# fusiyuan2010/CSC

Hardware: AMD Instinct MI355X
Metric: encode MB/s (10^6 input bytes / wall-clock) on enwik9 stand-in, -m3 -d64m; stream bit-exact vs reference (higher is better)
Workload: dtype u8/u32 (byte + 32-bit integer work; 12-bit probabilities, 64-bit range-coder low)

## Files before the change

csc_amd/csrc/csc_kernels.hip:

```cpp
#include <hip/hip_runtime.h>
#include <stdint.h>
#include <stdlib.h>

#include "csc_device.h"
#include "csc_tables.h"

namespace cscmi {

#define DEV __device__ __forceinline__
#define GLOBAL_AS __attribute__((address_space(1)))
typedef GLOBAL_AS uint8_t gu8;
typedef GLOBAL_AS uint16_t gu16;
typedef GLOBAL_AS uint32_t gu32;
typedef uint32_t __attribute__((ext_vector_type(4))) raw_vec4;
typedef GLOBAL_AS raw_vec4 gvec4;
#define UNI(x) ((uint32_t)__builtin_amdgcn_readfirstlane((int)(x)))

#ifndef CSCMI_TU
#define CSCMI_TU 0
#endif
static __device__ __constant__ uint32_t d_p2bits[512];
static __device__ __constant__ uint32_t d_logtable[513];

__device__ static const uint32_t kDltIndex[5] = {1, 2, 3, 4, 8};
// ... 9 lines not shown
struct DpShared {
    uint32_t cmd, idle;
    uint32_t dec;
    uint32_t price_done, relax_done;
    uint32_t ins_done, erep_done;
    uint32_t lp_int;
    uint32_t abort, gate;
    uint32_t wpos0, pos0, aplimit, limit0, stage_base, stage_end;
    uint32_t bstat[2];
    DpEdge e[2];
    uint16_t st_lit[64], st_p1[64];
    uint32_t e2[4][8];
    uint32_t er[4][8];
};
struct EncLds {
    uint32_t P[P_COUNT + 4];
    uint16_t p2b[512];
    uint32_t len_price[32], len_price_old[32];
    uint32_t rep[4];
    union {
        uint32_t cd2[kDpWaves][32];
        struct { uint32_t cd2_row0[32]; uint32_t cmp_pos[16], cmp_lim[16], cmp_res[16]; };
    };
    uint32_t rp42[kDpWaves][4];
    uint32_t rg_price[256], rg_dist[256];
    uint32_t rg_rep[256 * 4];
    uint16_t rg_back[256];
    uint8_t rg_state[256];
    union {
        struct {
            uint32_t fin_dist[kAPLimit + 1];
            uint16_t fin_back[kAPLimit + 2];
            union {
                uint16_t fin_next[kAPLimit + 2];
                struct { uint32_t appt_price[256], appt_dist[256]; };
            };
            uint8_t fin_lit[kAPLimit + 3];
        };
        uint32_t fin2[(kAPLimit + 1) * 2];
        struct { uint16_t trie_next[300 * 26]; uint8_t trie_sym[304]; };
        struct {
            uint2 tok[kTokRing];
            uint32_t pipe_cmd, pipe_ack, tok_head, tok_tail;
            uint32_t hand[16];
        };
    };
    DpShared dp;
    uint32_t stage[(kMinBlock + 64) / 4];
};

struct Sc {
    EncState *S;
    EncLds *L;
    void *X;
    struct CoderQ *Q;
    uint32_t q_head, q_room;
    gu8 *wnd;
    uint32_t wnd_size, vld_rge;
    gu32 *ht2, *ht3, *ht6, *bt_head, *bt_nodes, *p_lit, *p_delta, *mfbuf;
    uint32_t ht6_off, bth_off;
    bool fast_ht;
    uint32_t pr_off, pr_rmask, pr_pol;
    uint32_t gm6, gm2, gm3, gmb, gslot;
    uint32_t ht_bits, ht_width, ht_low, ht_cyc, bt_bits, bt_size, bt_cyc, good_len;
    uint32_t lz_good_len, lz_bt_cyc, lz_ht_cyc;
    uint32_t bt_pos, pos, wnd_curpos;
    uint32_t state, ctx, lp_rebuild_int;
    uint64_t rc_low;
    uint32_t rc_range, rc_cache, rc_cachesize, rc_size, bc_size, bc_curbits, bc_curval, bsize;
    gu8 *rc_buf, *bc_buf, *arena, *swapbuf;
    uint32_t arena_used, arena_cap, error;
    uint32_t lane;
    uint32_t stage_base, stage_end;
    uint32_t cand_len_v, cand_dist_v;
    uint32_t wv, dp_seq, dp_idle, dp_seq_seen;
    uint32_t st_find, st_slide, st_bt, st_lit, st_match;
    uint32_t pipe_ok, piped, tok_headl, tok_tail_seen, pipe_seq, pair_ok;
#ifdef CSCMI_TIMERS
    unsigned long long tm[16];
#endif
};

#ifdef CSCMI_TIMERS
#define TM_DECL unsigned long long tm__ = __builtin_readcyclecounter()
#define TM_ADD(c, k) do { unsigned long long n__ = __builtin_readcyclecounter(); (c).tm[k] += n__ - tm__; tm__ = n__; } while (0)
#define TM_RESET tm__ = __builtin_readcyclecounter()
#ifdef CSCMI_TIMERS_FINE
#define TMF_ADD(c, k) TM_ADD(c, k)
#else
#define TMF_ADD(c, k) do {} while (0)
#endif
#else
#define TMF_ADD(c, k) do {} while (0)
#define TM_DECL do {} while (0)
#define TM_ADD(c, k) do {} while (0)
#define TM_RESET do {} while (0)
#endif

DEV uint32_t umin(uint32_t a, uint32_t b) { return a < b ? a : b; }
DEV uint64_t uni64(uint64_t v) { return ((uint64_t)UNI((uint32_t)(v >> 32)) << 32) | UNI((uint32_t)v); }
template <class T> DEV T *uni_gptr(T *p) { return (T *)(uintptr_t)uni64((uint64_t)(uintptr_t)p); }
DEV void sc_uniform(Sc &c)
{
    c.S = uni_gptr(c.S); c.wnd = uni_gptr(c.wnd); c.wnd_size = UNI(c.wnd_size); c.vld_rge = UNI(c.vld_rge);
    c.ht2 = uni_gptr(c.ht2); c.ht3 = uni_gptr(c.ht3); c.ht6 = uni_gptr(c.ht6); c.bt_head = uni_gptr(c.bt_head); c.bt_nodes = uni_gptr(c.bt_nodes);
    c.p_lit = uni_gptr(c.p_lit); c.p_delta = uni_gptr(c.p_delta); c.mfbuf = uni_gptr(c.mfbuf);
    c.ht6_off = UNI(c.ht6_off); c.bth_off = UNI(c.bth_off);
    c.ht_bits = UNI(c.ht_bits); c.ht_width = UNI(c.ht_width); c.ht_low = UNI(c.ht_low); c.ht_cyc = UNI(c.ht_cyc);
    c.bt_bits = UNI(c.bt_bits); c.bt_size = UNI(c.bt_size); c.bt_cyc = UNI(c.bt_cyc); c.good_len = UNI(c.good_len);
    c.lz_good_len = UNI(c.lz_good_len); c.lz_bt_cyc = UNI(c.lz_bt_cyc); c.lz_ht_cyc = UNI(c.lz_ht_cyc);
    c.bt_pos = UNI(c.bt_pos); c.pos = UNI(c.pos); c.wnd_curpos = UNI(c.wnd_curpos);
    c.state = UNI(c.state); c.ctx = UNI(c.ctx); c.lp_rebuild_int = UNI(c.lp_rebuild_int);
    c.rc_low = uni64(c.rc_low); c.rc_range = UNI(c.rc_range); c.rc_cache = UNI(c.rc_cache); c.rc_cachesize = UNI(c.rc_cachesize);
    c.rc_size = UNI(c.rc_size); c.bc_size = UNI(c.bc_size); c.bc_curbits = UNI(c.bc_curbits); c.bc_curval = UNI(c.bc_curval); c.bsize = UNI(c.bsize);
    c.rc_buf = uni_gptr(c.rc_buf); c.bc_buf = uni_gptr(c.bc_buf); c.arena = uni_gptr(c.arena); c.swapbuf = uni_gptr(c.swapbuf);
    c.arena_used = UNI(c.arena_used); c.arena_cap = UNI(c.arena_cap); c.error = UNI(c.error);
    c.stage_base = UNI(c.stage_base); c.stage_end = UNI(c.stage_end);
    c.wv = UNI(c.wv); c.dp_seq = UNI(c.dp_seq); c.dp_idle = UNI(c.dp_idle); c.dp_seq_seen = UNI(c.dp_seq_seen);
    c.st_find = UNI(c.st_find); c.st_slide = UNI(c.st_slide); c.st_bt = UNI(c.st_bt); c.st_lit = UNI(c.st_lit); c.st_match = UNI(c.st_match);
    c.q_head = UNI(c.q_head); c.q_room = UNI(c.q_room);
}

DEV void wave_fence() { __builtin_amdgcn_fence(__ATOMIC_SEQ_CST, "workgroup"); }
DEV uint32_t rdlane(uint32_t v, uint32_t lane) { return (uint32_t)__builtin_amdgcn_readlane((int)v, (int)lane); }
DEV uint32_t wrlane(uint32_t val, uint32_t lane, uint32_t old) { return (threadIdx.x & 63u) == lane ? val : old; }

DEV uint64_t load8u(const gu8 *p)
{
    uintptr_t a = (uintptr_t)p;
    uint32_t sh = (uint32_t)a & 3u;
    const gu32 *q = (const gu32 *)(a & ~(uintptr_t)3);
    uint32_t d0 = q[0], d1 = q[1], d2 = q[2];
    uint32_t lo = __builtin_amdgcn_alignbyte(d1, d0, sh);
    uint32_t hi = __builtin_amdgcn_alignbyte(d2, d1, sh);
    return ((uint64_t)hi << 32) | lo;
}
DEV uint32_t ldb(const gu8 *p) { return UNI((uint32_t)*p); }

DEV uint64_t stage_load8(const uint32_t *stage, uint32_t byte_idx)
{
    uint32_t sh = byte_idx & 3u;
    const uint32_t *q = stage + (byte_idx >> 2);
    uint32_t d0 = q[0], d1 = q[1], d2 = q[2];
    uint32_t lo = __builtin_amdgcn_alignbyte(d1, d0, sh);
    uint32_t hi = __builtin_amdgcn_alignbyte(d2, d1, sh);
    return ((uint64_t)hi << 32) | lo;
}


__device__ __noinline__ void lanes_copy16(gvec4 *d4, const gvec4 *s4, uint32_t n16)
{
    for (uint32_t i = threadIdx.x & 63u; i < n16; i += 64) d4[i] = s4[i];
}
__device__ __noinline__ void lanes_copy8(gu8 *dst, const gu8 *src, uint32_t n)
{
    for (uint32_t t = threadIdx.x & 63u; t < n; t += 64) dst[t] = src[t];
}
__device__ __noinline__ void lanes_fill32(gu32 *dst, uint32_t n, uint32_t v)
{
    for (uint32_t t = threadIdx.x & 63u; t < n; t += 64) dst[t] = v;
}
__device__ __noinline__ void lanes_stage(uint8_t *sb, const gu8 *src, uint32_t first, uint32_t end)
{
    for (uint32_t t = first + (threadIdx.x & 63u); t < end; t += 64) sb[t] = src[t];
}
DEV void emit_block(Sc &c, uint32_t kind, const gu8 *buf, uint32_t size)
{
    uint32_t need = 16 + ((size + 15) & ~15u);
    if (c.arena_used + need > c.arena_cap) { c.error = ERR_ARENA_FULL; return; }
    gu8 *dst = c.arena + c.arena_used;
    wave_fence();
    ((gu32 *)dst)[0] = kind; ((gu32 *)dst)[1] = size;
    lanes_copy16((gvec4 *)(dst + 16), (const gvec4 *)buf, (size + 15) >> 4);
    c.arena_used += need;
}

constexpr uint32_t kCoderQ = 4096;
constexpr uint32_t kPDumpE = P_COUNT + 3;
struct CoderQ {
    uint32_t pub, tail, done, pad;
    uint32_t e[kCoderQ];
};
DEV void q_publish(Sc &c)
{
    __builtin_amdgcn_fence(__ATOMIC_RELEASE, "workgroup", "local");
    *(volatile __attribute__((address_space(3))) uint32_t *)&c.Q->pub = c.q_head;
}
DEV void q_publish_to(Sc &c, uint32_t to)
{
    __builtin_amdgcn_fence(__ATOMIC_RELEASE, "workgroup", "local");
    *(volatile __attribute__((address_space(3))) uint32_t *)&c.Q->pub = to;
}
constexpr uint32_t ERR_QUEUE_STALL = 0x40200000u;
DEV uint32_t q_wait_room(Sc &c, uint32_t need)
{
    uint32_t used, spins = 0;
    if (__builtin_expect(c.error != 0, 0)) return 0;
    while ((used = c.q_head - UNI(*(volatile __attribute__((address_space(3))) uint32_t *)&c.Q->tail)) > kCoderQ - need) {
        __builtin_amdgcn_s_sleep(2);
        if (++spins > (1u << 24)) { if (!c.error) c.error = ERR_QUEUE_STALL | (used & 0xFFFFu); return 0; }
    }
    return used;
}
DEV void q_push(Sc &c, uint32_t e)
{
    if (__builtin_expect(c.q_room == 0, 0)) {
        q_publish(c);
        c.q_room = umin(kCoderQ - 64u - q_wait_room(c, 128u), 256u);
    }
    c.Q->e[c.q_head & (kCoderQ - 1)] = e;
    c.q_head++; c.q_room--;
}

DEV void q_push_bits(Sc &c, uint32_t pold, uint32_t bit, uint32_t n, uint32_t from = 0)
{
    if (__builtin_expect(c.q_room < n, 0)) {
        q_publish(c);
        c.q_room = umin(kCoderQ - 64u - q_wait_room(c, 128u), 256u);
    }
    const uint32_t k = c.lane - from;
    c.Q->e[(c.q_head + (k < n ? k : 63u)) & (kCoderQ - 1)] = 0x80000000u | (bit ? 0x1000u : 0u) | pold;
    c.q_head += n; c.q_room -= n;
}

DEV void rc_put(Sc &c, uint32_t byte)
{
    c.rc_buf[c.rc_size++] = (uint8_t)byte;
    if (c.rc_size == c.bsize) { emit_block(c, 1, c.rc_buf, c.bsize); c.rc_size = 0; }
}

DEV void rc_shift_low(Sc &c)
{
    uint32_t low32 = (uint32_t)c.rc_low, top = (uint32_t)(c.rc_low >> 32);
    if (low32 < 0xFF000000u || top != 0) {
        uint32_t temp = c.rc_cache;
        do {
            rc_put(c, (temp + top) & 0xFF);
            temp = 0xFF;
        } while (--c.rc_cachesize != 0);
        c.rc_cache = low32 >> 24;
    }
    c.rc_cachesize++;
    c.rc_low = (uint64_t)(low32 << 8);
}

DEV void rc_code(Sc &c, uint32_t v, uint32_t p)
{
    if (c.Q) { q_push(c, 0x80000000u | (v ? 0x1000u : 0u) | p); return; }
    const uint32_t bound = (c.rc_range >> 12) * p;
    c.rc_low += v ? 0u : bound;
    c.rc_range = v ? bound : c.rc_range - bound;
    if (__builtin_expect(c.rc_range < (1u << 24), 0)) { c.rc_range <<= 8; rc_shift_low(c); }
}
DEV uint32_t p_update(uint32_t v, uint32_t p) { return v ? p + ((0xFFFu - p) >> 5) : p - (p >> 5); }

DEV void enc_bit_lds(Sc &c, uint32_t v, uint32_t idx)
{
    uint32_t p = UNI(c.L->P[idx]);
    c.L->P[idx] = p_update(v, p);
    rc_code(c, v, p);
}

DEV void bc_put(Sc &c, uint32_t byte)
{
    c.bc_buf[c.bc_size++] = (uint8_t)byte;
    if (c.bc_size == c.bsize) { emit_block(c, 0, c.bc_buf, c.bsize); c.bc_size = 0; }
}

DEV void enc_direct16(Sc &c, uint32_t val, uint32_t len)
{
    if (c.Q) { q_push(c, 0x40000000u | (len << 16) | (val & 0xFFFFu)); return; }
    c.bc_curval = (c.bc_curval << len) | val;
    c.bc_curbits += len;
    while (c.bc_curbits >= 8) {
        bc_put(c, (c.bc_curval >> (c.bc_curbits - 8)) & 0xFF);
        c.bc_curbits -= 8;
    }
}
DEV void enc_direct(Sc &c, uint32_t v, uint32_t l)
{
    if (l <= 16) enc_direct16(c, v, l);
    else { enc_direct16(c, v >> 16, l - 16); enc_direct16(c, v & 0xFFFF, 16); }
}

DEV void coder_flush(Sc &c)
{
    if (c.Q) { q_push(c, 0x20000000u); q_publish(c); return; }
    for (int i = 0; i < 5; i++) rc_shift_low(c);
    c.rc_size++;
    bc_put(c, (c.bc_curval << (8 - c.bc_curbits)) & 0xFF);
    bc_put(c, 0);
    emit_block(c, 1, c.rc_buf, c.rc_size);
    emit_block(c, 0, c.bc_buf, c.bc_size);
    c.rc_low = 0; c.rc_range = 0xFFFFFFFFu; c.rc_cachesize = 1; c.rc_cache = 0;
    c.rc_size = c.bc_size = 0; c.bc_curbits = c.bc_curval = 0;
}


DEV uint32_t bit_price(const Sc &c, uint32_t v, uint32_t p)
{
    return UNI(c.L->p2b[(v ? p : 4096u - p) >> 3]);
}
DEV uint32_t lds_price(const Sc &c, uint32_t v, uint32_t idx) { return bit_price(c, v, UNI(c.L->P[idx])); }

DEV void encode_int(Sc &c, uint32_t num)
{
    uint32_t slot = num ? 31u - (uint32_t)__builtin_clz(num) : 0u;
    enc_direct(c, slot, 5);
    if (slot == 0) enc_direct(c, num, 1);
    else enc_direct(c, num - (1u << slot), slot);
}

DEV void encode_matchlen_1(Sc &c, uint32_t len)
{
    if (len < 16) {
        uint32_t base;
        if (len < 8) { enc_bit_lds(c, 0, P_LEN_SLOT); base = P_LEN_X1; }
// ... 370 lines not shown
```

csc_amd/csrc/csc_kernels_blocks.inc:

```


DEV uint32_t e89_xswap(uint32_t x)
{
    x <<= 7;
    return (x >> 24) | (((x >> 16) & 0xFFu) << 8) | (((x >> 8) & 0xFFu) << 16) | ((x & 0xFFu) << (24 - 7));
}
DEV void flt_forward_e89(Sc &c, gu8 *src, uint32_t size)
{
    uint32_t next_ok = 0;
    for (uint32_t base = 0; base + 5 < size; base += 64) {
        uint32_t j0 = base + c.lane;
        bool cand = false;
        if (j0 + 5 < size) cand = (src[j0] & 0xFEu) == 0xE8u;
        uint64_t m = __ballot(cand);
        while (m) {
            uint32_t bit = (uint32_t)__builtin_ctzll(m);
            m &= m - 1;
            uint32_t j = base + bit;
            if (j < next_ok) continue;
            next_ok = j + 4;
            uint64_t v = load8u(src + j + 1);
            uint32_t x = UNI((uint32_t)v) - 0xFF000000u;
            if (x < 0x02000000u) {
                x = (x + (j + 5)) & 0x01FFFFFFu;
                x = e89_xswap(x) + 0xFF000000u;
                src[j + 1] = (uint8_t)x; src[j + 2] = (uint8_t)(x >> 8);
                src[j + 3] = (uint8_t)(x >> 16); src[j + 4] = (uint8_t)(x >> 24);
            }
        }
        wave_fence();
    }
}

DEV void flt_forward_delta(Sc &c, gu8 *src, uint32_t size, uint32_t chn)
{
    if (size < 512) return;
    gu8 *copy = c.swapbuf;
    for (uint32_t t = c.lane; t < size; t += 64) copy[t] = src[t];
    wave_fence();
    for (uint32_t j = c.lane; j < size; j += 64) {
        uint32_t ch = j % chn, idx = j / chn;
        uint32_t dst = idx;
        for (uint32_t k = 0; k < ch; k++) dst += (size - k + chn - 1) / chn;
        uint32_t prev = 0;
        if (idx > 0) prev = copy[j - chn];
        else if (ch > 0) {
            uint32_t nprev = (size - (ch - 1) + chn - 1) / chn;
            prev = copy[(ch - 1) + (nprev - 1) * chn];
        }
        src[dst] = (uint8_t)(copy[j] - prev);
    }
    wave_fence();
}

DEV uint32_t umax16(uint32_t a, uint32_t b) { return a > b ? a : b; }
DEV uint32_t flt_compose(uint32_t A, uint32_t B) { return __builtin_amdgcn_perm(0u, B, A); }
DEV uint32_t flt_forward_dict(Sc &c, gu8 *src, uint32_t size)
{
    if (size < 16384) return 0;
    EncLds *L = c.L;
    EncState *S = c.S;
    gu8 *dst = c.swapbuf;
    const uint32_t n5 = size - 5;
    for (uint32_t i = c.lane; i < 300 * 26; i += 64) L->trie_next[i] = S->trie_next[i];
    for (uint32_t i = c.lane; i < 300; i += 64) L->trie_sym[i] = S->trie_sym[i];
    uint32_t s_in = 0, dst_size = 0, p = 0;
    const uint64_t lower = (1ull << c.lane) - 1ull;
    uint64_t v8n = load8u(src + c.lane);
    for (uint32_t base = 0; base < n5; base += 64) {
        const uint32_t i = base + c.lane;
        const bool valid = i < n5;
        const uint64_t v8 = v8n;
        if (base + 64 < n5) v8n = load8u(src + i + 64);
        const uint32_t b = (uint32_t)v8 & 0xFFu;
        uint32_t sym = 0, adv = 1;
        if (valid && b >= 'a' && b <= 'z') {
            uint32_t node = 0;
            for (uint32_t j = 0; j < 8;) {
                const uint32_t idx = ((uint32_t)(v8 >> (8u * j)) & 0xFFu) - 'a';
                if (idx > 25) break;
                const uint32_t nx = L->trie_next[node * 26 + idx];
                if (nx == 0) break;
                node = nx;
                j++;
                const uint32_t ws = L->trie_sym[node];
                if (ws) { sym = ws; adv = j; }
            }
        }
        uint32_t inc = valid ? (((adv - 1u) & 3u) | 0x02010000u) : 0x03020100u;
#pragma unroll
        for (int o = 1; o < 64; o <<= 1) {
            const uint32_t t = (uint32_t)__shfl_up((int)inc, o);
            inc = (int)c.lane >= o ? flt_compose(t, inc) : inc;
        }
        const uint32_t prev = (uint32_t)__shfl_up((int)inc, 1);
        const uint32_t sb = c.lane == 0 ? s_in : (prev >> (8u * s_in)) & 3u;
        const bool mine = valid && sb == 0;
        const uint64_t on = __ballot(mine);
        const bool two = mine && sym == 0 && b >= 0x82;
        const uint64_t m2 = __ballot(two);
        const uint32_t off = dst_size + (uint32_t)__builtin_popcountll(on & lower) + (uint32_t)__builtin_popcountll(m2 & lower);
        if (mine) {
            if (sym) dst[off] = (uint8_t)sym;
            else if (two) { dst[off] = 254; dst[off + 1] = (uint8_t)b; }
            else dst[off] = (uint8_t)b;
        }
        dst_size += (uint32_t)__builtin_popcountll(on) + (uint32_t)__builtin_popcountll(m2);
        const uint32_t vcount = umin(64u, n5 - base);
        s_in = (rdlane(inc, vcount - 1) >> (8u * s_in)) & 3u;
        p = base + vcount + s_in;
    }
    wave_fence();
    for (uint32_t i = p; i < size; i++) {
        uint32_t b = ldb(src + i);
        if (b >= 0x82) { dst[dst_size++] = 254; dst[dst_size++] = (uint8_t)b; }
        else dst[dst_size++] = (uint8_t)b;
    }
    if ((double)dst_size > (double)size * 0.82) return 0;
    wave_fence();
    {
        const uint32_t full = dst_size & ~15u, up = (size + 15u) & ~15u;
        const gvec4 *s4 = (const gvec4 *)dst;
        gvec4 *d4 = (gvec4 *)src;
        raw_vec4 blanks; blanks.x = blanks.y = blanks.z = blanks.w = 0x20202020u;
        for (uint32_t t = c.lane * 16u; t < full; t += 1024u) d4[t >> 4] = s4[t >> 4];
        for (uint32_t t = full + c.lane; t < umin(full + 16u, size); t += 64) src[t] = t < dst_size ? dst[t] : (uint8_t)0x20;
        for (uint32_t t = full + 16u + c.lane * 16u; t + 16u <= size; t += 1024u) d4[t >> 4] = blanks;
        for (uint32_t t = umax16(full + 16u, size & ~15u) + c.lane; t < size; t += 64) src[t] = (uint8_t)0x20;
        (void)up;
    }
    wave_fence();
    return 1;
}

#if CSCMI_TU != 2
template <int WHICH>
__device__ __noinline__ uint32_t flt_dp4_nl(EncState *S, gu8 *swapbuf, gu8 *src, uint32_t size, uint32_t chn)
{
    Sc c;
    c.S = S; c.L = &g_lds4.base; c.swapbuf = swapbuf; c.lane = threadIdx.x & 63u;
    if (WHICH == 0) { flt_forward_e89(c, src, size); return 0; }
    if (WHICH == 1) return flt_forward_dict(c, src, size);
    flt_forward_delta(c, src, size, chn);
    return 0;
}
#endif
template <int PARSER, int FORM>
DEV void enc_compress_block(Sc &c, gu8 *src, uint32_t size, uint32_t type)
{
    if (size == 0) return;
    uint32_t mode = c.S->lz_mode;
    const bool is_dlt = type >= DT_DLT && type < DT_DLT + 5;
    if (type == DT_NORMAL) {
        encode_int(c, type);
    } else if (type == DT_EXE) {
        encode_int(c, type);
#if CSCMI_TU != 2
        if (FORM == 2) (void)flt_dp4_nl<0>(uni_gptr(c.S), uni_gptr(c.swapbuf), uni_gptr(src), UNI(size), 0);
        else
#endif
        flt_forward_e89(c, src, size);
    } else if (type == DT_ENGTXT) {
        TM_DECL;
        uint32_t ok;
#if CSCMI_TU != 2
        if (FORM == 2) ok = UNI(flt_dp4_nl<1>(uni_gptr(c.S), uni_gptr(c.swapbuf), uni_gptr(src), UNI(size), 0));
        else
#endif
        ok = flt_forward_dict(c, src, size);
        TM_ADD(c, 8);
        c.S->dict_result = ok;
        if (ok) { encode_int(c, type); encode_int(c, size); }
        else encode_int(c, DT_NORMAL);
    } else if (type == DT_FAST) {
        encode_int(c, DT_NORMAL);
    } else if (type == DT_BAD || type == DT_ENTROPY || is_dlt) {
        encode_int(c, type);
        mode = 5;
    } else {
        c.error = ERR_BAD_TYPE;
        return;
    }
    lz_encode_normal<PARSER, FORM>(c, src, size, mode);
    if (type == DT_BAD) compress_bad(c, src, size);
    else if (type == DT_ENTROPY) compress_literals(c, src, size);
    else if (is_dlt) {
#if CSCMI_TU != 2
        if (FORM == 2) (void)flt_dp4_nl<2>(uni_gptr(c.S), uni_gptr(c.swapbuf), uni_gptr(src), UNI(size), kDltIndex[type - DT_DLT]);
        else
#endif
        flt_forward_delta(c, src, size, kDltIndex[type - DT_DLT]);
        compress_rle(c, src, size);
    }
}

DEV bool dev_is_duplicate(Sc &c, const gu8 *src, uint32_t size)
{
    wave_fence();
    const uint32_t wpos = c.wnd_curpos, vld = c.vld_rge, wsz = c.wnd_size;
    for (uint32_t base = 0; base < size; base += 64) {
        const uint32_t i = base + c.lane;
        bool hit = false;
        if (i < size) {
            const uint64_t v = load8u(src + i);
            const uint32_t lo = (uint32_t)v, hi2 = (uint32_t)(v >> 32) & 0xFFFFu;
            if ((hash2_of(lo) & 15u) == 0) {
                const uint32_t hv = hash6_mul(lo, hi2);
                const uint32_t limit = size - i;
                uint32_t d[2] = {0xFFFFFFFFu, 0xFFFFFFFFu};
                if (c.ht_width) d[0] = c.pos - c.ht6[(size_t)(hv >> (32 - c.ht_bits)) * c.ht_width];
                if (c.bt_head) d[1] = c.pos - c.bt_head[hv >> (32 - c.bt_bits)];
#pragma unroll
                for (int k = 0; k < 2; k++) {
                    const uint32_t dist = d[k];
                    if (dist >= vld) continue;
                    const uint32_t cp = wpos >= dist ? wpos - dist : wpos + wsz - dist;
                    const uint32_t climit = umin(limit, wsz - cp);
                    if (climit <= 18) continue;
                    const gu8 *q = c.wnd + cp;
                    const bool e0 = load8u(src + i) == load8u(q), e1 = load8u(src + i + 8) == load8u(q + 8);
                    const uint64_t t2 = (load8u(src + i + 16) ^ load8u(q + 16)) & 0xFFFFFFull;
                    hit = hit || (e0 && e1 && t2 == 0);
                }
            }
        }
        if (__ballot(hit)) return true;
    }
    return false;
}

struct SegWalk { uint32_t csize, i, blk, last_type, last_begin, last_size, bpb; };
DEV void seg_start(SegWalk &w, uint32_t csize) { w.csize = csize; w.i = 0; w.blk = 0; w.last_type = DT_NORMAL; w.last_begin = 0; w.last_size = 0; w.bpb = 0; }
DEV bool seg_next(Sc &c, SegWalk &w, uint32_t &type, uint32_t &off, uint32_t &size, uint32_t &tail)
{
    EncState *S = c.S;
    const gu8 *src = (const gu8 *)S->inbuf;
    const uint32_t ff = S->filt_flags;
    const BlockInfo *binfo = S->binfo;
    while (w.i < w.csize) {
        const uint32_t cur = umin(kMinBlock, w.csize - w.i);
        uint32_t this_type = DT_NORMAL;
        if (ff) {
            this_type = UNI(binfo[w.blk].type);
            if (this_type != DT_SKIP) w.bpb = UNI(binfo[w.blk].bpb);
        }
        if (this_type == DT_SKIP) this_type = w.last_type;
        if (this_type != DT_NORMAL) {
            if (this_type == DT_EXE && !(ff & 4u)) this_type = DT_NORMAL;
            else if (this_type == DT_ENGTXT && !(ff & 2u)) this_type = DT_NORMAL;
            else if (this_type >= DT_DLT && !(ff & 1u)) this_type = DT_NORMAL;
        }
        if (this_type >= DT_DLT && (double)UNI(binfo[w.blk].dlt_bpb[this_type - DT_DLT]) >= w.bpb * 0.95) this_type = DT_NORMAL;
        if (this_type >= DT_NO_LZ && dev_is_duplicate(c, src + w.i, cur)) this_type = DT_NORMAL;
        const bool close = (w.last_type != this_type || w.last_size + cur > S->raw_blocksize) && w.last_size;
        if (w.last_type != this_type || w.last_size + cur > S->raw_blocksize) {
            type = w.last_type; off = w.last_begin; size = w.last_size; tail = 0;
            w.last_begin = w.i;
            w.last_size = 0;
        }
        w.last_type = this_type;
        w.last_size += cur;
        w.i += cur;
        w.blk++;
        if (close) return true;
    }
    if (w.last_size) { type = w.last_type; off = w.last_begin; size = w.last_size; tail = 1; w.last_size = 0; return true; }
    return false;
}

DEV void sc_load_regs(Sc &c, EncState *S, EncLds *L)
{
    const GLOBAL_AS EncState *G = (const GLOBAL_AS EncState *)S;
    c.S = S; c.L = L; c.X = nullptr; c.Q = nullptr; c.q_head = 0; c.q_room = 0;
    c.lane = threadIdx.x & 63;
    c.wnd = (gu8 *)G->wnd; c.wnd_size = G->wnd_size; c.vld_rge = G->vld_rge;
    c.ht2 = (gu32 *)G->ht2; c.ht3 = (gu32 *)G->ht3; c.ht6 = (gu32 *)G->ht6; c.bt_head = (gu32 *)G->bt_head; c.bt_nodes = (gu32 *)G->bt_nodes;
    c.p_lit = (gu32 *)G->p_lit; c.p_delta = (gu32 *)G->p_delta; c.swapbuf = (gu8 *)G->swapbuf;
    c.mfbuf = (gu32 *)G->mfbuf;
    c.ht6_off = kHT2Size + kHT3Size;
    c.bth_off = c.ht6_off + (G->ht_width << G->ht_bits);
    {
        uint32_t wd = G->ht_width < G->lz_ht_cyc ? G->ht_width : G->lz_ht_cyc;
        c.gm6 = c.lane < wd ? 0xFFFFFFFFu : 0u;
        c.gm2 = c.lane == 32 ? 0xFFFFFFFFu : 0u;
        c.gm3 = c.lane == 33 ? 0xFFFFFFFFu : 0u;
        c.gmb = (c.lane == 34 && G->bt_head) ? 0xFFFFFFFFu : 0u;
// ... 505 lines not shown
```

csc_amd/csrc/csc_kernels_lz.inc:

```

DEV void lz_encode_nonlit(Sc &c, uint32_t ulen, uint32_t udist)
{
    EncLds *L = c.L;
    if (udist <= 4) {
        if (ulen == 1 && udist == 1) encode_rep0len1(c);
        else {
            encode_rep_match(c, udist - 1, ulen - 2);
            uint32_t d = UNI(L->rep[udist - 1]);
            for (uint32_t k = udist - 1; k > 0; k--) L->rep[k] = UNI(L->rep[k - 1]);
            L->rep[0] = d;
        }
    } else {
        encode_match(c, udist - 5, ulen - 2);
        uint32_t r0 = UNI(L->rep[0]), r1 = UNI(L->rep[1]), r2 = UNI(L->rep[2]);
        L->rep[3] = r2; L->rep[2] = r1; L->rep[1] = r0; L->rep[0] = udist - 4;
    }
}

typedef volatile __attribute__((address_space(3))) uint32_t lds_vu32;
DEV uint32_t lds_vload(uint32_t *p) { return UNI(*(lds_vu32 *)p); }
DEV void lds_vstore(uint32_t *p, uint32_t v) { *(lds_vu32 *)p = v; }
DEV void lds_release() { __builtin_amdgcn_fence(__ATOMIC_RELEASE, "workgroup"); }
DEV void lds_acquire() { __builtin_amdgcn_fence(__ATOMIC_ACQUIRE, "workgroup"); }

// ... 184 lines not shown
            encode_match(c, nd - 5, next - i - 2);
            c.ctx = UNI(L->fin_lit[next - 1]);
        }
        i = next;
    }
    L->rep[c.lane & 3u] = L->rg_rep[(end & 255u) * 4 + (c.lane & 3u)];
}

DEV void lz_compress_advanced(Sc &c, uint32_t size)
{
    EncLds *L = c.L;
    size = UNI(size);
    for (uint32_t i = 0; i < size;) {
        sc_uniform(c);
        i = UNI(i);
        uint32_t a0l = 1, a0d = 0;
        uint32_t apcur = 0, apend = 1;
        const uint32_t aplimit = umin(kAPLimit, size - i);
        for (;;) {
            TM_DECL;
            const uint32_t sidx = c.wnd_curpos - c.stage_base + 16;
            uint64_t v9 = stage_load8(L->stage, sidx - 1);
            const uint32_t b01 = UNI((uint32_t)v9), b45 = UNI((uint32_t)(v9 >> 32));
            const uint32_t lit_ctx = c.wnd_curpos ? (b01 & 0xFFu) : 0u;
            const uint32_t cur_lit = (b01 >> 8) & 0xFFu;
            const MfPre pre = mf_pre(c, (b01 >> 8) | (b45 << 24), b45 >> 8);
            const uint32_t lk = c.lane & 7, lcc = cur_lit | 0x100u;
            const uint32_t plit_raw = c.p_lit[lit_ctx * 256 + (lcc >> (8 - lk))];
            const uint32_t slot = apcur & 255u;
            uint32_t cur_state, r0, r1, r2, r3, base_price;
            if (apcur) {
                cur_state = UNI(L->rg_state[slot]);
                r0 = UNI(L->rg_rep[slot * 4 + 0]); r1 = UNI(L->rg_rep[slot * 4 + 1]);
                r2 = UNI(L->rg_rep[slot * 4 + 2]); r3 = UNI(L->rg_rep[slot * 4 + 3]);
                base_price = UNI(L->rg_price[slot]);
                L->fin_dist[apcur] = UNI(L->rg_dist[slot]);
                L->fin_back[apcur] = (uint16_t)UNI(L->rg_back[slot]);
            } else {
                cur_state = c.state;
                r0 = UNI(L->rep[0]); r1 = UNI(L->rep[1]); r2 = UNI(L->rep[2]); r3 = UNI(L->rep[3]);
                base_price = 0;
                L->rg_price[0] = 0;
                L->fin_back[0] = 0;
                L->rg_rep[0] = r0; L->rg_rep[1] = r1; L->rg_rep[2] = r2; L->rg_rep[3] = r3;
            }
            L->fin_lit[apcur] = (uint8_t)cur_lit;
            bool has1 = false;
            uint32_t p1 = 0, lane_dist = 0, lane_price = 0, t_lit0 = 0;
            if (apcur < aplimit) {
                TM_ADD(c, 4);
                mf_find_priced(c, cur_state, c.wnd_curpos, size - i - apcur, pre, r0, r1, r2, r3, a0l, a0d, has1, p1, lane_dist, lane_price, t_lit0);
                TM_RESET;
            }
            uint32_t exit_kind = 0;
            if (apcur == 0 && a0d == 0) exit_kind = 2;
            else if (apcur == aplimit) exit_kind = 1;
            else if (a0l == 1 && apcur + 1 == apend) exit_kind = 2;
            else {
                if (apcur + 1 >= apend) { L->rg_price[apend & 255u] = 0xFFFFFFFFu; apend++; }
                if (a0l >= c.lz_good_len || (a0l > 1 && a0l + apcur >= aplimit)) exit_kind = 3;
            }
            if (exit_kind) {
                lz_ap_backward(c, apcur);
                i += apcur;
                if (exit_kind == 2) {
                    encode_literal(c, cur_lit);
                    c.wnd_curpos++;
                    i++;
                } else if (exit_kind == 3) {
                    lz_encode_nonlit(c, a0l, a0d);
                    mf_slide_pos(c, c.wnd_curpos, a0l, size - i);
                    i += a0l;
                    c.wnd_curpos += a0l;
                    c.ctx = stage_byte(c, c.wnd_curpos - 1);
                }
                TM_ADD(c, 6);
                break;
            }
            uint32_t cprice;
            {
                uint32_t bit = (lcc >> (7 - lk)) & 1;
                uint32_t pr = L->p2b[(bit ? plit_raw : 4096u - plit_raw) >> 3];
                pr += dpp_row_shr<1>(0, pr);
                pr += dpp_row_shr<2>(0, pr);
                pr += dpp_row_shr<4>(0, pr);
                cprice = rdlane(pr, 7) + t_lit0;
            }
            const uint32_t s1slot = (apcur + 1) & 255u;
            uint32_t nprice = UNI(L->rg_price[s1slot]);
            uint32_t n_dist = 0xFFFFFFFFu;
            if (cprice + base_price < nprice) { nprice = cprice + base_price; n_dist = 0; }
            if (has1 && p1 + base_price < nprice) { nprice = p1 + base_price; n_dist = 1; }
            if (n_dist != 0xFFFFFFFFu) {
                L->rg_dist[s1slot] = n_dist;
                L->rg_back[s1slot] = (uint16_t)apcur;
                L->rg_price[s1slot] = nprice;
                L->rg_state[s1slot] = (uint8_t)((cur_state * 4 + (n_dist ? 2 : 0)) & 0x3F);
                L->rg_rep[s1slot * 4 + 0] = r0; L->rg_rep[s1slot * 4 + 1] = r1;
                L->rg_rep[s1slot * 4 + 2] = r2; L->rg_rep[s1slot * 4 + 3] = r3;
            }
            const uint32_t len = a0l;
            if (apcur + len >= apend) {
                for (uint32_t t0 = apend; t0 <= apcur + len; t0 += 64) L->rg_price[umin(t0 + c.lane, apcur + len) & 255u] = 0xFFFFFFFFu;
                apend = apcur + len + 1;
            }
            for (uint32_t l0 = 2; l0 <= len; l0 += 64) {
                const uint32_t ll = l0 + c.lane;
                const bool in = ll <= len;
                const uint32_t lli = in ? ll : 2u;
                const uint32_t ad = l0 == 2 ? lane_dist : L->appt_dist[lli];
                const uint32_t pr = l0 == 2 ? lane_price : L->appt_price[lli];
                const uint32_t t0 = (apcur + ll) & 255u;
                const uint32_t was = L->rg_price[t0];
                const bool win = in & (ad != 0) & (pr + base_price < was);
                const uint32_t t = win ? t0 : slot;
                L->rg_dist[t] = ad;
                L->rg_back[t] = (uint16_t)apcur;
                L->rg_price[t] = pr + base_price;
                const bool isrep = ad <= 4;
                const uint32_t rsel0 = L->cd2[c.wv][(ad - 1) & 3u];
                const uint32_t ns = (cur_state * 4 + (isrep ? 3u : 1u)) & 0x3F;
                const uint32_t n0 = isrep ? rsel0 : ad - 4;
                const uint32_t n1 = (isrep && ad == 1) ? r1 : r0;
                const uint32_t n2 = (isrep && ad <= 2) ? r2 : r1;
                const uint32_t n3 = (isrep && ad <= 3) ? r3 : r2;
                L->rg_state[t] = (uint8_t)ns;
                L->rg_rep[t * 4 + 0] = n0; L->rg_rep[t * 4 + 1] = n1; L->rg_rep[t * 4 + 2] = n2; L->rg_rep[t * 4 + 3] = n3;
            }
            apcur++;
            c.wnd_curpos++;
            TM_ADD(c, 5);
        }
    }
}

DEV void lz_compress_advanced_dp4(Sc &c, uint32_t size);
DEV void d4_master_call(Sc &c, uint32_t size);
DEV void lz_compress_advanced_bt(Sc &c, uint32_t size);
DEV void bt_parser_call(Sc &c, uint32_t size);
DEV bool bt_ok(const Sc &c, uint32_t size);
DEV void lz_compress_normal_hp(Sc &c, uint32_t size, bool lazy);
DEV void hp_parser_call(Sc &c, uint32_t size, bool lazy);
DEV bool hp_ok(const Sc &c);

template <int PARSER, int FORM>
DEV void lz_encode_normal(Sc &c, const gu8 *src, uint32_t size, uint32_t lz_mode)
{
    const bool two_waves = PARSER == 2 && lz_mode != 5 && c.pipe_ok;
    if (two_waves) pipe_begin(c);
    for (uint32_t i = 0; i < size;) {
        uint32_t cur = umin(c.wnd_size - c.wnd_curpos, size - i);
        cur = umin(cur, kMinBlock);
        {
            gu8 *dst = c.wnd + c.wnd_curpos;
            const gu8 *s = src + i;
            TM_DECL;
            lanes_copy8(dst, s, cur);
            wave_fence();
            c.stage_base = c.wnd_curpos;
            c.stage_end = c.wnd_curpos + cur + 40;
            uint32_t first = c.wnd_curpos >= 16 ? 0u : 16u - c.wnd_curpos;
            uint8_t *sb = (uint8_t *)c.L->stage;
            lanes_stage(sb, c.wnd + c.wnd_curpos - 16, first, cur + 16 + 48);
            TM_ADD(c, 9);
        }
        if (lz_mode == 5) {
            mf_slide_pos_fast(c, c.wnd_curpos, cur);
            c.wnd_curpos += cur;
        } else {
            if (PARSER == 3) {
                if (FORM == 3 && bt_ok(c, cur)) bt_parser_call(c, cur);
                else if (FORM == 2 && c.pair_ok && c.pos < 0xFFFF0000u) d4_master_call(c, cur);
                else lz_compress_advanced(c, cur);
            }
            else if (FORM == 4 && hp_ok(c)) hp_parser_call(c, cur, lz_mode == 2);
            else lz_compress_normal(c, cur, lz_mode == 2);
        }
        if (c.wnd_curpos >= c.wnd_size) c.wnd_curpos = 0;
        i += cur;
    }
    if (lz_mode != 5) {
        if (c.piped) tok_push(c, TOK_NONLIT_KEEPCTX | (2u << 16), 64 + 5);
        else encode_match(c, 64, 0);
    }
    if (two_waves) pipe_end(c);
}
```

Baseline: 2.912.

## Vectorize window/stage copy and restructure dictionary filter with DPP scan and packed trie

```diff
diff --git a/csc_amd/csrc/csc_kernels.hip b/csc_amd/csrc/csc_kernels.hip
--- a/csc_amd/csrc/csc_kernels.hip
+++ b/csc_amd/csrc/csc_kernels.hip
@@ -185,17 +185,79 @@
 {
     for (uint32_t i = threadIdx.x & 63u; i < n16; i += 64) d4[i] = s4[i];
 }
-__device__ __noinline__ void lanes_copy8(gu8 *dst, const gu8 *src, uint32_t n)
-{
-    for (uint32_t t = threadIdx.x & 63u; t < n; t += 64) dst[t] = src[t];
+DEV raw_vec4 load16u(const gu8 *p)
+{
+    const uintptr_t a = (uintptr_t)p;
+    const uint32_t sh = (uint32_t)a & 3u;
+    const gu32 *q = (const gu32 *)(a & ~(uintptr_t)3);
+    const uint32_t d0 = q[0], d1 = q[1], d2 = q[2], d3 = q[3], d4 = sh ? q[4] : 0u;
+    raw_vec4 v;
+    v.x = __builtin_amdgcn_alignbyte(d1, d0, sh); v.y = __builtin_amdgcn_alignbyte(d2, d1, sh);
+    v.z = __builtin_amdgcn_alignbyte(d3, d2, sh); v.w = __builtin_amdgcn_alignbyte(d4, d3, sh);
+    return v;
+}
+constexpr int kCopyBatch = 8;
+DEV void lanes_copy16_far(gvec4 *__restrict__ d4, const gvec4 *__restrict__ s4, uint32_t n16)
+{
+    const uint32_t lane = threadIdx.x & 63u;
+    for (uint32_t u0 = 0; u0 < n16; u0 += 64u * kCopyBatch) {
+        raw_vec4 v[kCopyBatch];
+#pragma unroll
+        for (int k = 0; k < kCopyBatch; k++) v[k] = s4[umin(u0 + 64u * k + lane, n16 - 1u)];
+#pragma unroll
+        for (int k = 0; k < kCopyBatch; k++) {
+            const uint32_t u = u0 + 64u * k + lane;
+            if (u < n16) d4[u] = v[k];
+        }
+    }
+}
+constexpr int kStageBatch = 4;
+__device__ __noinline__ void lanes_copy_stage(gu8 *__restrict__ wnd, const gu8 *__restrict__ src, uint8_t *sb, uint32_t wpos, uint32_t first, uint32_t n)
+{
+    const uint32_t lane = threadIdx.x & 63u;
+    gu8 *dst = wnd + wpos;
+    const uint32_t j = lane < 16u ? lane : n + lane;
+    const bool around = lane >= 16u || lane >= first;
+    uint8_t ab = 0;
+    if (around) ab = (wnd + wpos - 16)[j];
+    const uint32_t sn16 = n >> 4;
+    const uint32_t st = (sn16 << 4) + lane;
+    uint8_t stb = 0;
+    if (lane < 16u && st < n) stb = src[st];
+    const uint32_t head = umin(n, (16u - (wpos & 15u)) & 15u), cn16 = (n - head) >> 4;
+    const uint32_t ct = head + (cn16 << 4) + (lane - 16u);
+    uint8_t hb = 0;
+    if (lane < head) hb = src[lane];
+    else if (lane >= 16u && lane < 32u && ct < n) hb = src[ct];
+    typedef __attribute__((address_space(3), aligned(8))) raw_vec4 lvec4;
+    static_assert(alignof(EncLds) % 8 == 0 && offsetof(EncLds, stage) % 8 == 0, "the stage's 16-byte units are written as two aligned 8-byte halves");
+    typedef __attribute__((address_space(3))) uint8_t lu8;
+    lu8 *sl = (lu8 *)sb;
+    lvec4 *s4 = (lvec4 *)(sl + 16);
+    gvec4 *d4 = (gvec4 *)(dst + head);
+    const gu8 *csrc = src + head;
+    for (uint32_t u0 = lane; u0 < sn16; u0 += 64u * kStageBatch) {
+        raw_vec4 v[kStageBatch];
+#pragma unroll
+        for (int k = 0; k < kStageBatch; k++) v[k] = load16u(src + umin(u0 + 64u * k, sn16 - 1u) * 16u);
+#pragma unroll
+        for (int k = 0; k < kStageBatch; k++) if (u0 + 64u * k < sn16) s4[u0 + 64u * k] = v[k];
+    }
+    if (around) sl[j] = ab;
+    if (lane < 16u && st < n) sl[16u + st] = stb;
+    for (uint32_t u0 = lane; u0 < cn16; u0 += 64u * kStageBatch) {
+        raw_vec4 v[kStageBatch];
+#pragma unroll
+        for (int k = 0; k < kStageBatch; k++) v[k] = load16u(csrc + umin(u0 + 64u * k, cn16 - 1u) * 16u);
+#pragma unroll
+        for (int k = 0; k < kStageBatch; k++) if (u0 + 64u * k < cn16) d4[u0 + 64u * k] = v[k];
+    }
+    if (lane < head) dst[lane] = hb;
+    else if (lane >= 16u && lane < 32u && ct < n) dst[ct] = hb;
 }
 __device__ __noinline__ void lanes_fill32(gu32 *dst, uint32_t n, uint32_t v)
 {
     for (uint32_t t = threadIdx.x & 63u; t < n; t += 64) dst[t] = v;
-}
-__device__ __noinline__ void lanes_stage(uint8_t *sb, const gu8 *src, uint32_t first, uint32_t end)
-{
-    for (uint32_t t = first + (threadIdx.x & 63u); t < end; t += 64) sb[t] = src[t];
 }
 DEV void emit_block(Sc &c, uint32_t kind, const gu8 *buf, uint32_t size)
 {
diff --git a/csc_amd/csrc/csc_kernels_blocks.inc b/csc_amd/csrc/csc_kernels_blocks.inc
--- a/csc_amd/csrc/csc_kernels_blocks.inc
+++ b/csc_amd/csrc/csc_kernels_blocks.inc
@@ -55,61 +55,108 @@
 
 DEV uint32_t umax16(uint32_t a, uint32_t b) { return a > b ? a : b; }
 DEV uint32_t flt_compose(uint32_t A, uint32_t B) { return __builtin_amdgcn_perm(0u, B, A); }
+constexpr int kDictW = 2;
+constexpr uint32_t kFltIdent = 0x03020100u;
+constexpr uint32_t kTrieEdges = 300 * 26;
+template <int CTRL, int ROWS> DEV uint32_t flt_dpp(uint32_t v) { return (uint32_t)__builtin_amdgcn_update_dpp((int)kFltIdent, (int)v, CTRL, ROWS, 0xF, false); }
+DEV uint32_t flt_mbcnt(uint64_t m) { return __builtin_amdgcn_mbcnt_hi((uint32_t)(m >> 32), __builtin_amdgcn_mbcnt_lo((uint32_t)m, 0u)); }
+#define FLT_SCAN(CTRL, ROWS) _Pragma("unroll") for (int g = 0; g < W; g++) inc[g] = flt_compose(flt_dpp<CTRL, ROWS>(inc[g]), inc[g])
 DEV uint32_t flt_forward_dict(Sc &c, gu8 *src, uint32_t size)
 {
+    size = UNI(size);
+    src = uni_gptr(src);
     if (size < 16384) return 0;
+    constexpr int W = kDictW;
     EncLds *L = c.L;
-    EncState *S = c.S;
-    gu8 *dst = c.swapbuf;
+    const GLOBAL_AS EncState *G = (const GLOBAL_AS EncState *)uni_gptr(c.S);
+    gu8 *dst = uni_gptr(c.swapbuf);
     const uint32_t n5 = size - 5;
-    for (uint32_t i = c.lane; i < 300 * 26; i += 64) L->trie_next[i] = S->trie_next[i];
-    for (uint32_t i = c.lane; i < 300; i += 64) L->trie_sym[i] = S->trie_sym[i];
-    uint32_t s_in = 0, dst_size = 0, p = 0;
-    const uint64_t lower = (1ull << c.lane) - 1ull;
-    uint64_t v8n = load8u(src + c.lane);
-    for (uint32_t base = 0; base < n5; base += 64) {
-        const uint32_t i = base + c.lane;
-        const bool valid = i < n5;
-        const uint64_t v8 = v8n;
-        if (base + 64 < n5) v8n = load8u(src + i + 64);
-        const uint32_t b = (uint32_t)v8 & 0xFFu;
-        uint32_t sym = 0, adv = 1;
-        if (valid && b >= 'a' && b <= 'z') {
-            uint32_t node = 0;
-            for (uint32_t j = 0; j < 8;) {
-                const uint32_t idx = ((uint32_t)(v8 >> (8u * j)) & 0xFFu) - 'a';
-                if (idx > 25) break;
-                const uint32_t nx = L->trie_next[node * 26 + idx];
-                if (nx == 0) break;
-                node = nx;
-                j++;
-                const uint32_t ws = L->trie_sym[node];
-                if (ws) { sym = ws; adv = j; }
+    {
+        const gu16 *tn = (const gu16 *)G->trie_next;
+        const gu8 *ts = (const gu8 *)G->trie_sym;
+        for (uint32_t i0 = c.lane; i0 < kTrieEdges; i0 += 64u * 8u) {
+            uint32_t nx[8], sy[8];
+#pragma unroll
+            for (int k = 0; k < 8; k++) nx[k] = tn[umin(i0 + 64u * k, kTrieEdges - 1u)];
+#pragma unroll
+            for (int k = 0; k < 8; k++) sy[k] = ts[nx[k]];
+#pragma unroll
+            for (int k = 0; k < 8; k++)
+                if (i0 + 64u * k < kTrieEdges) L->trie_next[i0 + 64u * k] = (uint16_t)((nx[k] && sy[k]) ? nx[k] | ((sy[k] - 0x81u) << 9) : nx[k]);
+        }
+    }
+    uint32_t s_in = 0, dst_size = 0;
+    gu8 *const dump = dst + 3u * (size_t)size + c.lane;
+    const uint32_t sh = (uint32_t)(uintptr_t)(src + c.lane) & 3u;
+    uint32_t rawn[W][3];
+#pragma unroll
+    for (int g = 0; g < W; g++) {
+        const gu32 *q = (const gu32 *)((uintptr_t)(src + umin(64u * g + c.lane, n5)) & ~(uintptr_t)3);
+        rawn[g][0] = q[0]; rawn[g][1] = q[1]; rawn[g][2] = q[2];
+    }
+    for (uint32_t base = 0; base < n5; base += 64u * W) {
+        uint64_t v8[W];
+        uint32_t b[W], sym[W], adv[W], node[W], inc[W];
+        bool valid[W], go[W];
+#pragma unroll
+        for (int g = 0; g < W; g++)
+            v8[g] = ((uint64_t)__builtin_amdgcn_alignbyte(rawn[g][2], rawn[g][1], sh) << 32) | __builtin_amdgcn_alignbyte(rawn[g][1], rawn[g][0], sh);
+#pragma unroll
+        for (int g = 0; g < W; g++) {
+            const gu32 *q = (const gu32 *)((uintptr_t)(src + umin(base + 64u * (W + g) + c.lane, n5)) & ~(uintptr_t)3);
+            rawn[g][0] = q[0]; rawn[g][1] = q[1]; rawn[g][2] = q[2];
+        }
+#pragma unroll
+        for (int g = 0; g < W; g++) {
+            valid[g] = base + 64u * g + c.lane < n5;
+            b[g] = (uint32_t)v8[g] & 0xFFu;
+            sym[g] = 0; adv[g] = 1; node[g] = 0; go[g] = valid[g];
+        }
+        for (uint32_t j = 1; j <= 8; j++) {
+            uint32_t e[W];
+#pragma unroll
+            for (int g = 0; g < W; g++) {
+                const uint32_t idx = ((uint32_t)v8[g] & 0xFFu) - 'a';
+                go[g] = go[g] && idx <= 25u;
+                e[g] = L->trie_next[go[g] ? node[g] * 26u + idx : 0u];
+                v8[g] >>= 8;
             }
-        }
-        uint32_t inc = valid ? (((adv - 1u) & 3u) | 0x02010000u) : 0x03020100u;
-#pragma unroll
-        for (int o = 1; o < 64; o <<= 1) {
-            const uint32_t t = (uint32_t)__shfl_up((int)inc, o);
-            inc = (int)c.lane >= o ? flt_compose(t, inc) : inc;
-        }
-        const uint32_t prev = (uint32_t)__shfl_up((int)inc, 1);
-        const uint32_t sb = c.lane == 0 ? s_in : (prev >> (8u * s_in)) & 3u;
-        const bool mine = valid && sb == 0;
-        const uint64_t on = __ballot(mine);
-        const bool two = mine && sym == 0 && b >= 0x82;
-        const uint64_t m2 = __ballot(two);
-        const uint32_t off = dst_size + (uint32_t)__builtin_popcountll(on & lower) + (uint32_t)__builtin_popcountll(m2 & lower);
-        if (mine) {
-            if (sym) dst[off] = (uint8_t)sym;
-            else if (two) { dst[off] = 254; dst[off + 1] = (uint8_t)b; }
-            else dst[off] = (uint8_t)b;
-        }
-        dst_size += (uint32_t)__builtin_popcountll(on) + (uint32_t)__builtin_popcountll(m2);
-        const uint32_t vcount = umin(64u, n5 - base);
-        s_in = (rdlane(inc, vcount - 1) >> (8u * s_in)) & 3u;
-        p = base + vcount + s_in;
-    }
+            bool any = false;
+#pragma unroll
+            for (int g = 0; g < W; g++) {
+                const uint32_t nx = e[g] & 511u, f = e[g] >> 9;
+                go[g] = go[g] && nx != 0;
+                node[g] = go[g] ? nx : node[g];
+                const bool word = go[g] && f != 0;
+                sym[g] = word ? 0x81u + f : sym[g];
+                adv[g] = word ? j : adv[g];
+                any = any || go[g];
+            }
+            if (!__ballot(any)) break;
+        }
+#pragma unroll
+        for (int g = 0; g < W; g++) inc[g] = valid[g] ? (((adv[g] - 1u) & 3u) | 0x02010000u) : kFltIdent;
+        FLT_SCAN(0x111, 0xF); FLT_SCAN(0x112, 0xF); FLT_SCAN(0x114, 0xF); FLT_SCAN(0x118, 0xF);
+        FLT_SCAN(0x142, 0xA); FLT_SCAN(0x143, 0xC);
+        uint32_t s = s_in;
+#pragma unroll
+        for (int g = 0; g < W; g++) {
+            const uint32_t prev = flt_dpp<0x138, 0xF>(inc[g]);
+            const uint32_t sb = (prev >> (8u * s)) & 3u;
+            const bool mine = valid[g] && sb == 0;
+            const uint64_t on = __ballot(mine);
+            const bool two = mine && sym[g] == 0 && b[g] >= 0x82;
+            const uint64_t m2 = __ballot(two);
+            const uint32_t off = dst_size + flt_mbcnt(on) + flt_mbcnt(m2);
+            gu8 *const a1 = mine ? dst + off : dump, *const a2 = two ? dst + off + 1 : dump;
+            *a1 = (uint8_t)(sym[g] ? sym[g] : two ? 254u : b[g]);
+            *a2 = (uint8_t)b[g];
+            dst_size += (uint32_t)__builtin_popcountll(on) + (uint32_t)__builtin_popcountll(m2);
+            s = (rdlane(inc[g], 63) >> (8u * s)) & 3u;
+        }
+        s_in = s;
+    }
+    const uint32_t p = n5 + s_in;
     wave_fence();
     for (uint32_t i = p; i < size; i++) {
         uint32_t b = ldb(src + i);
@@ -119,19 +166,18 @@
     if ((double)dst_size > (double)size * 0.82) return 0;
     wave_fence();
     {
-        const uint32_t full = dst_size & ~15u, up = (size + 15u) & ~15u;
-        const gvec4 *s4 = (const gvec4 *)dst;
+        const uint32_t full = dst_size & ~15u;
         gvec4 *d4 = (gvec4 *)src;
         raw_vec4 blanks; blanks.x = blanks.y = blanks.z = blanks.w = 0x20202020u;
-        for (uint32_t t = c.lane * 16u; t < full; t += 1024u) d4[t >> 4] = s4[t >> 4];
+        lanes_copy16_far(d4, (const gvec4 *)dst, full >> 4);
         for (uint32_t t = full + c.lane; t < umin(full + 16u, size); t += 64) src[t] = t < dst_size ? dst[t] : (uint8_t)0x20;
         for (uint32_t t = full + 16u + c.lane * 16u; t + 16u <= size; t += 1024u) d4[t >> 4] = blanks;
         for (uint32_t t = umax16(full + 16u, size & ~15u) + c.lane; t < size; t += 64) src[t] = (uint8_t)0x20;
-        (void)up;
     }
     wave_fence();
     return 1;
 }
+#undef FLT_SCAN
 
 #if CSCMI_TU != 2
 template <int WHICH>
diff --git a/csc_amd/csrc/csc_kernels_lz.inc b/csc_amd/csrc/csc_kernels_lz.inc
--- a/csc_amd/csrc/csc_kernels_lz.inc
+++ b/csc_amd/csrc/csc_kernels_lz.inc
@@ -360,16 +360,14 @@
         uint32_t cur = umin(c.wnd_size - c.wnd_curpos, size - i);
         cur = umin(cur, kMinBlock);
         {
-            gu8 *dst = c.wnd + c.wnd_curpos;
             const gu8 *s = src + i;
             TM_DECL;
-            lanes_copy8(dst, s, cur);
-            wave_fence();
             c.stage_base = c.wnd_curpos;
             c.stage_end = c.wnd_curpos + cur + 40;
             uint32_t first = c.wnd_curpos >= 16 ? 0u : 16u - c.wnd_curpos;
             uint8_t *sb = (uint8_t *)c.L->stage;
-            lanes_stage(sb, c.wnd + c.wnd_curpos - 16, first, cur + 16 + 48);
+            lanes_copy_stage(c.wnd, s, sb, c.wnd_curpos, first, cur);
+            wave_fence();
             TM_ADD(c, 9);
         }
         if (lz_mode == 5) {
```

New measurement: 3.070 (median of 6 runs). 1.05x the previous value.
